# GuanxingLu/ManiGaussian

Hardware: AMD Instinct MI355X
Metric: Gaussians rasterized/sec (fwd+bwd), 128x128, 32 feat-ch; HBM GB/s vs peak (higher is better)
Workload: dtype f32

## Files before the change

### manigaussian_amd/csrc/mgs_render_dense.hip

```cpp
#include "mgs_render_common.h"

namespace mgs {

constexpr int TRACE_EVENTS = 24;
__device__ unsigned long long g_trace[512 * 16 * TRACE_EVENTS];
#define MGS_TRACE(ev)                                                                                      \
  do {                                                                                                     \
    if ((r.dbg & 256) && lane == 0 && blockIdx.x < 512 && (ev) < TRACE_EVENTS)                              \
      g_trace[((size_t)blockIdx.x * 16 + w) * TRACE_EVENTS + (ev)] = __builtin_amdgcn_s_memtime();         \
  } while (0)

template <int F, bool FAST, bool EXACT, int NW, int CHS, bool TWO>
__global__ void __launch_bounds__(NW * 64, TWO ? 4 : 1)
coop_fwd_pairs_kernel(RenderArgs r, const uint2* __restrict__ ranges, const uint32_t* __restrict__ point_list,
                      float* __restrict__ T_end, float* __restrict__ T_mid,
                      uint32_t* __restrict__ last_pos, float* __restrict__ partial, uint32_t* __restrict__ surv,
                      size_t surv_stride, uint2* __restrict__ nsurv, float* __restrict__ final_T,
                      uint32_t* __restrict__ last_chunk, float* __restrict__ out_color, float* __restrict__ out_feat,
                      uint32_t* __restrict__ round_base, uint32_t pool, uint32_t* __restrict__ flags, int nblocks,
                      uint64_t* host_status, uint32_t status_tag, unsigned long long* hs_fail_mark) {
  static_assert(CHS == 64, "a chunk is two 32-lane groups of the Gaussian-major backward");
  using f32x16 = __attribute__((ext_vector_type(16))) float;
  constexpr int NCH = F + 3;
  constexpr bool MF = F >= 16;
  constexpr int NT = MF ? (F + 31) / 32 : 0;
  constexpr int NVF = MF ? 0 : F;
  constexpr int NP = NW / 2;
  constexpr int NS = 2;
  constexpr int NSTEP = CHS / 2;
  constexpr int TRS = 33;
  constexpr int NOWN = (NCH + NW - 1) / NW;
  constexpr uint32_t ROUND = NW * CHS;
  constexpr uint32_t FSTEP = NW * 64;
  constexpr int FILLK = 3;
  constexpr int TRR = NT * 32 + 3;
  __shared__ float trs[MF ? NW * TRR * TRS : 1];
  __shared__ uint32_t lastcc[NW];
  __shared__ float4 recP[NW][CHS / 4 * 2 * 3];
  __shared__ uint32_t sid[NW * CHS];
  __shared__ float4 rowq[NW][NS][CHS];
  __shared__ float rowf[NVF > 0 ? NW * NS * CHS * NVF : 1];
  __shared__ float Tp[2][NW][64];
  __shared__ unsigned long long red_last[64];
  __shared__ uint32_t cnt[2][FILLK * NW];
  __shared__ uint32_t rbase[2];
  constexpr uint32_t RBH = 16;
  __shared__ uint32_t rb_hist[RBH];
  const int tid = threadIdx.x, lane = tid & 63;
  const int w = __builtin_amdgcn_readfirstlane(tid >> 6);
  if (blockIdx.x == 0 && tid == 0 && hs_fail_mark) *hs_fail_mark = 0ull;
  const int pr = w >> 1, hh = w & 1;
  const int k_ = lane >> 5, pl_ = lane & 31;
  int tile, sub;
  map_block(blockIdx.x, tile, sub);
  if (tile >= r.tiles_x * r.tiles_y) return;
  const PixBlk p = pix_blk(r, tile, sub, lane);
  const int pixq_ = 32 * hh + pl_;
  const int pixq = pixq_, k = k_, pl = pl_;
  const PixBlk pq = pix_blk(r, tile, sub, pixq);
  const int pixx_ = 32 * (hh ^ k) + pl;
  const int pixx = pixx_;
  const bool insidex = pix_blk(r, tile, sub, pixx).inside;
  const uint2 rng = ranges[tile];
  const bool use_feat = (F > 0) && r.include_feature;
  const auto feat_rsrc = __builtin_amdgcn_make_buffer_rsrc(const_cast<float*>(r.feats), 0, 0xffffffffu, 0x00020000);
  uint32_t* __restrict__ my_rounds = round_base + round_entry(rng.x, tile, sub, 0);
  bool overflow = false;
  uint32_t* my_surv = surv + (size_t)sub * surv_stride + rng.x;

  float Tround = 1.0f;
  uint32_t my_vis = 0;
  float my_Tf = 1.0f;
  if (w == 0) red_last[lane] = (unsigned long long)__float_as_uint(1.0f);
  uint32_t my_lastcc = 0xffffffffu;
  MGS_TRACE(0);

  uint32_t next = rng.x;
  uint32_t qhead = 0;
  uint32_t qtail = 0;
  uint32_t cbase = 0;
  uint32_t fill = 0;
  uint32_t round = 0;

  const bool allocator = tid == (NW - 1) * 64;
  const bool static0 = (uint32_t)nblocks <= 1024u && (uint32_t)nblocks * (uint32_t)NW <= pool;
  const uint32_t dyn_base = static0 ? (uint32_t)nblocks * (uint32_t)NW : 0u;
  for (;; round++) {
    int k = k_, pl = pl_, pixq = pixq_, pixx = pixx_;
    asm volatile("" : "+v"(k), "+v"(pl), "+v"(pixq), "+v"(pixx));
    uint32_t b0 = 0;
    const bool more = next < rng.y || qtail > qhead;
    if (allocator && more) {
      if (static0 && round == 0) b0 = ((uint32_t)tile * 4u + (uint32_t)sub) * (uint32_t)NW;
      else b0 = dyn_base + atomicAdd(&flags[FLAG_CHUNKS_USED], (uint32_t)NW);
    }
    while (qtail - qhead < ROUND && next < rng.y) {
      uint32_t idd[FILLK], rk[FILLK];
      float4 a0[FILLK], a1[FILLK];
      {
#pragma unroll
        for (int kf = 0; kf < FILLK; kf++) {
          const uint32_t e = next + (uint32_t)kf * FSTEP + (uint32_t)tid;
          idd[kf] = e < rng.y ? point_list[e] : 0xffffffffu;
        }
#pragma unroll
        for (int kf = 0; kf < FILLK; kf++) {
          a0[kf] = make_float4(0, 0, 0, 0); a1[kf] = make_float4(0, 0, -1.f, -1.f);
          if (idd[kf] != 0xffffffffu) { a0[kf] = r.rec[2 * (size_t)idd[kf]]; a1[kf] = r.rec[2 * (size_t)idd[kf] + 1]; }
        }
#pragma unroll
        for (int kf = 0; kf < FILLK; kf++) {
          const bool sk = idd[kf] != 0xffffffffu && cull_ok<EXACT>(a0[kf], a1[kf], p);
          const unsigned long long sm = ballot(sk);
          rk[kf] = sk ? (uint32_t)__builtin_popcountll(sm & ((1ull << lane) - 1ull)) : 0xffffffffu;
          if (lane == 0) cnt[fill & 1][kf * NW + w] = (uint32_t)__builtin_popcountll(sm);
        }
      }
      __syncthreads();
      const uint32_t v = lane < FILLK * NW ? cnt[fill & 1][lane] : 0u;
      const uint32_t incl = wave_incl_scan_add_u32(v);
      const uint32_t total = bcast_lane_u32(incl, 63);
#pragma unroll
      for (int kf = 0; kf < FILLK; kf++) {
        const uint32_t base = bcast_lane_u32(incl - v, kf * NW + w);
        if (rk[kf] != 0xffffffffu) {
          const uint32_t n = qtail + base + rk[kf];
          my_surv[n] = idd[kf];
          if (round == 0 && n < ROUND) {
            const uint32_t e = n & (CHS - 1);
            float* rp = reinterpret_cast<float*>(&recP[n / CHS][0]) + (((e >> 2) * 2 + (e & 1)) * 12 + ((e >> 1) & 1));
            rp[0] = a0[kf].x; rp[2] = a0[kf].y; rp[4] = a0[kf].z; rp[6] = a0[kf].w; rp[8] = a1[kf].x; rp[10] = a1[kf].y;
            sid[n] = idd[kf];
          }
        }
      }
      qtail += total;
      next += FILLK * FSTEP;
      fill++;
    }
    if (allocator && more) {
      rbase[round & 1] = b0;
      if (round < RBH) rb_hist[round] = b0;
      my_rounds[4 * (size_t)round] = b0;
    }
    MGS_TRACE(1 + 8 * round);
    __syncthreads();
    MGS_TRACE(2 + 8 * round);
    const uint32_t avail = qtail - qhead;
    const bool exhausted = !(next < rng.y);
    uint32_t nchunk = exhausted ? (avail + CHS - 1) / CHS : avail / CHS;
    nchunk = min(nchunk, (uint32_t)NW);
    if (nchunk == 0) break;

    struct Rec3 { float4 XY, CC, ZO; };
    auto rec3_of = [&](uint32_t buf, int j) -> Rec3 {
      return Rec3{recP[buf][(2 * j + k) * 3], recP[buf][(2 * j + k) * 3 + 1], recP[buf][(2 * j + k) * 3 + 2]};
    };
    auto alpha2_rec = [&](const Rec3& R) -> f32x2 {
      const float4 XY = R.XY, CC = R.CC, ZO = R.ZO;
      const f32x2 dx = f32x2{XY.x, XY.y} - pq.pxf, dy = f32x2{XY.z, XY.w} - pq.pyf;
      const f32x2 power = gauss_power2v(f32x2{CC.x, CC.y}, f32x2{CC.z, CC.w}, f32x2{ZO.x, ZO.y}, dx, dy);
      const f32x2 G = exp2_<FAST>(power);
      const f32x2 oG = f32x2{ZO.z, ZO.w} * G;
      const float a0 = fminf(0.99f, oG.x), a1 = fminf(0.99f, oG.y);
      return f32x2{((power.x > 0.0f) || (a0 < 1.0f / 255.0f)) ? 0.f : a0, ((power.y > 0.0f) || (a1 < 1.0f / 255.0f)) ? 0.f : a1};
    };
    auto alpha2_of = [&](uint32_t buf, int j) -> f32x2 { return alpha2_rec(rec3_of(buf, j)); };
    float al[NSTEP];
    uint32_t nmy[NS];
#pragma unroll
    for (int q = 0; q < NS; q++) {
      const uint32_t ci = (uint32_t)pr + (uint32_t)q * NP;
      const bool hasq = ci < nchunk;
      nmy[q] = hasq ? min((uint32_t)CHS, avail - ci * CHS) : 0u;
      if (q == 0) {
#pragma unroll
        for (int s = 0; s < NSTEP; s++) al[s] = 0.f;
      }
      float tp = 1.0f;
      if (hasq) {
        float4 rq = make_float4(0, 0, 0, __uint_as_float(0u));
        float fv[NVF > 0 ? NVF : 1];
#pragma unroll
        for (int i = 0; i < (NVF > 0 ? NVF : 1); i++) fv[i] = 0.f;
        const bool valid = (uint32_t)lane < nmy[q];
        float* rp = reinterpret_cast<float*>(&recP[ci][0]) + (((lane >> 2) * 2 + (lane & 1)) * 12 + ((lane >> 1) & 1));
        int tile_ = tile;
        asm volatile("" : "+s"(tile_));
        const uint32_t gbase = gauss_base(r, tile_);
        auto colour_row = [&](uint32_t id) {
          const uint32_t gid = gauss_of(gbase, id);
          const uint32_t cid = r.colors_per_view ? id : gid;
          rq = make_float4(r.colors[(size_t)cid * 3], r.colors[(size_t)cid * 3 + 1], r.colors[(size_t)cid * 3 + 2],
                           __uint_as_float(gid));
          if constexpr (NVF > 0) {
            if (use_feat) {
#pragma unroll
              for (int i = 0; i < NVF; i++) fv[i] = r.feats[(size_t)gid * F + i];
            }
          }
        };
        if (round == 0) {
          if (valid) {
            colour_row(sid[ci * CHS + (uint32_t)lane]);
          } else {
            rp[0] = 0.f; rp[2] = 0.f; rp[4] = 0.f; rp[6] = 0.f; rp[8] = 0.f; rp[10] = 0.f;
            rq.w = __uint_as_float(gauss_of(gbase, sid[ci * CHS]));
          }
        } else {
          float4 g0 = make_float4(0, 0, 0, 0), g1 = make_float4(0, 0, -1.f, -1.f);
          if (valid) {
            const uint32_t id = my_surv[qhead + ci * CHS + (uint32_t)lane];
            g0 = r.rec[2 * (size_t)id]; g1 = r.rec[2 * (size_t)id + 1];
            colour_row(id);
          } else {
            rq.w = __uint_as_float(gauss_of(gbase, my_surv[qhead + ci * CHS]));
          }
          rp[0] = g0.x; rp[2] = g0.y; rp[4] = g0.z; rp[6] = g0.w; rp[8] = g1.x;
          rp[10] = valid ? g1.y : 0.f;
        }
        wave_lds_sync();
        if (q == 0) MGS_TRACE(3 + 8 * round);
        f32x2 tp2 = {1.0f, 1.0f};
        Rec3 Rn = rec3_of(ci, 0);
#pragma unroll
        for (int j = 0; j < NSTEP / 2; j++) {
          const Rec3 Rc = Rn;
          if (j + 1 < NSTEP / 2) Rn = rec3_of(ci, j + 1);
          const f32x2 a2 = alpha2_rec(Rc);
          if (q == 0) { al[2 * j] = a2.x; al[2 * j + 1] = a2.y; }
          tp2 = tp2 * (1.0f - a2);
        }
        tp = tp2.x * tp2.y;
        rowq[w][q][lane] = rq;
        if constexpr (NVF > 0) {
#pragma unroll
          for (int i = 0; i < NVF; i++) rowf[(((size_t)w * NS + q) * CHS + lane) * NVF + i] = fv[i];
        }
        float t0 = tp, t1 = tp;
        swap32(t0, t1);
        tp = t0 * t1;
      }
      if (k == 0) Tp[round & 1][ci][pixq] = tp;
    }
    MGS_TRACE(4 + 8 * round);
    __syncthreads();
    __builtin_amdgcn_s_waitcnt(0x0F70);
    MGS_TRACE(5 + 8 * round);
    const uint32_t rb = rbase[round & 1];
    if (rb + (uint32_t)NW > pool) { overflow = true; break; }
    float Tin[NS], Tnext = Tround;
#pragma unroll
    for (int q = 0; q < NS; q++) Tin[q] = Tround;
#pragma unroll
    for (int c2 = 0; c2 < NW; c2++) {
      const float t2 = Tp[round & 1][c2][pixx];
#pragma unroll
      for (int q = 0; q < NS; q++) Tin[q] = (c2 < pr + q * NP) ? Tin[q] * t2 : Tin[q];
      Tnext *= t2;
    }
#pragma unroll
    for (int q = 0; q < NS; q++) {
      const uint32_t ci = (uint32_t)pr + (uint32_t)q * NP;
      const bool hasq = ci < nchunk;
      const float Tpart = __uint_as_float(lane_xor<32>(__float_as_uint(Tin[q]), lane));
      float T = k ? Tpart : Tin[q];
      const bool live = hasq && pq.inside && !(T < 0.0001f);
      if (ballot(live) != 0) {
        const uint32_t n_my = nmy[q];
        float Cc[3] = {0.f, 0.f, 0.f};
        float Cv[NVF > 0 ? NVF : 1];
#pragma unroll
        for (int i = 0; i < (NVF > 0 ? NVF : 1); i++) Cv[i] = 0.f;
        f32x16 acc[NT > 0 ? NT : 1];
#pragma unroll
        for (int t = 0; t < (NT > 0 ? NT : 1); t++)
#pragma unroll
          for (int i = 0; i < 16; i++) acc[t][i] = 0.f;
        constexpr int BD = 4;
        float Bq[NT > 0 ? NT : 1][BD];
        uint32_t gnext = __float_as_uint(rowq[w][q][k].w);
        auto load_B = [&](int s) {
          const uint32_t gide = gnext;
          if (s + 1 < NSTEP) gnext = __float_as_uint(rowq[w][q][2 * (s + 1) + k].w);
#pragma unroll
          for (int t = 0; t < (NT > 0 ? NT : 1); t++) {
            const int ch = 32 * t + pl;
            if constexpr (MF)
              Bq[t][s % BD] = __uint_as_float(__builtin_amdgcn_raw_buffer_load_b32(
                  feat_rsrc, gide * (uint32_t)(F * 4) + (uint32_t)((ch < F ? ch : 0) * 4), 0, 0));
          }
        };
        if constexpr (MF) {
#pragma unroll
          for (int s = 0; s < BD; s++) load_B(s);
        }
        float Tc = live ? T : 0.f;
        uint32_t last = 0;
        float Tm = T;
        bool stop = false;
        constexpr int GS = 4;
#pragma unroll
        for (int g = 0; g < NSTEP / GS; g++) {
          if (g * GS == NSTEP / 2) Tm = T;
          stop = stop || (uint32_t)(2 * g * GS) >= n_my || ballot(Tc != 0.f) == 0;
          __builtin_amdgcn_sched_barrier(0);
          if (!stop) {
            f32x2 a2q = {0.f, 0.f};
#pragma unroll
            for (int u4 = 0; u4 < GS; u4++) {
              const int s = g * GS + u4;
              if (q != 0 && (u4 & 1) == 0) a2q = alpha2_of(ci, s >> 1);
              float a0 = (q == 0) ? al[s] : ((u4 & 1) ? a2q.y : a2q.x), a1 = a0;
              swap32(a0, a1);
              float wq[2];
              const float aa[2] = {a0, a1};
#pragma unroll
              for (int u = 0; u < 2; u++) {
                const float test_T = Tc * (1.0f - aa[u]);
                const bool term = test_T < 0.0001f;
                wq[u] = (term ? 0.f : aa[u]) * Tc;
                Tc = term ? 0.f : test_T;
                T = term ? T : test_T;
                last = wq[u] > 0.f ? (uint32_t)(2 * s + u) + 1u : last;
              }
              const float wk = k ? wq[1] : wq[0];
              const float4 rq = rowq[w][q][2 * s + k];
              Cc[0] += rq.x * wk; Cc[1] += rq.y * wk; Cc[2] += rq.z * wk;
              if constexpr (NVF > 0) {
#pragma unroll
                for (int i = 0; i < NVF; i++) Cv[i] += rowf[(((size_t)w * NS + q) * CHS + 2 * s + k) * NVF + i] * wk;
              }
              if constexpr (MF) {
#pragma unroll
                for (int t = 0; t < NT; t++) {
                  float bv = Bq[t][s % BD];
                  if constexpr (F % 32 != 0) bv = (32 * t + pl) < F ? bv : 0.f;
                  acc[t] = __builtin_amdgcn_mfma_f32_32x32x2f32(wk, bv, acc[t], 0, 0, 0);
                }
                if (s + BD < NSTEP) load_B(s + BD);
              }
            }
          }
        }
        if constexpr (MF) {
#pragma unroll
          for (int t = 0; t < NT; t++)
#pragma unroll
            for (int i = 0; i < BD; i++) asm volatile("" ::"v"(Bq[t][i]));
        }
        if (last <= 32u) Tm = T;
#pragma unroll
        for (int i = 0; i < 3; i++) Cc[i] += __uint_as_float(lane_xor<32>(__float_as_uint(Cc[i]), lane));
#pragma unroll
        for (int i = 0; i < NVF; i++) Cv[i] += __uint_as_float(lane_xor<32>(__float_as_uint(Cv[i]), lane));
        MGS_TRACE(6 + 8 * round);
        const size_t slot = (size_t)rb + (size_t)ci;
        float* pp = partial + slot * NCH * 64 + pixq;
        if (k == 0) {
          T_end[slot * 64 + pixq] = T;
          T_mid[slot * 64 + pixq] = Tm;
          last_pos[slot * 64 + pixq] = last;
#pragma unroll
          for (int i = 0; i < 3; i++) pp[i * 64] = Cc[i];
#pragma unroll
          for (int i = 0; i < NVF; i++) pp[(3 + i) * 64] = Cv[i];
        }
        if constexpr (MF) {
          float* tb = trs + (size_t)w * TRR * TRS;
#pragma unroll
          for (int t = 0; t < NT; t++)
#pragma unroll
            for (int i = 0; i < 16; i++)
              tb[(32 * t + pl) * TRS + (i & 3) + 8 * (i >> 2) + 4 * k] = acc[t][i];
          if (k == 0) {
#pragma unroll
            for (int i = 0; i < 3; i++) tb[(NT * 32 + i) * TRS + pl] = Cc[i];
          }
          wave_lds_sync();
#pragma unroll
          for (int c = 0; c < F / 2; c++) {
            const int ch = k * (F / 2) + c;
            pp[(3 + ch) * 64] = tb[ch * TRS + pl];
          }
          wave_lds_sync();
          my_lastcc = cbase + ci;
        }
        if (live) { my_vis = cbase + ci + 1; my_Tf = T; }
      }
    }
    MGS_TRACE(7 + 8 * round);
    Tround = Tnext;
    qhead += min(avail, nchunk * CHS);
    cbase += nchunk;
    if (ballot(insidex && !(Tround < 0.0001f)) == 0) break;
  }

  MGS_TRACE(TRACE_EVENTS - 3);
  if (my_vis > 0 && k == 0)
    atomicMax(&red_last[pixq], ((unsigned long long)my_vis << 32) | (unsigned long long)__float_as_uint(my_Tf));
  if constexpr (MF) { if (lane == 0) lastcc[w] = my_lastcc; }
  __syncthreads();
  const unsigned long long rl = red_last[lane];
  const uint32_t vis = (uint32_t)(rl >> 32);
  const float Tf = __uint_as_float((uint32_t)rl);
  float img[NOWN];
#pragma unroll
  for (int kk = 0; kk < NOWN; kk++) img[kk] = 0.f;
  const uint32_t vmax = wave_umax(vis);
  constexpr int NFLY = 8;
  static_assert(NW % NFLY == 0, "a batch of the final sum lies inside one round");
  for (uint32_t c0 = 0; c0 < vmax; c0 += NFLY) {
    float v[NFLY][NOWN];
    const uint32_t rr = c0 / NW;
    uint32_t rb0 = rb_hist[rr < RBH ? rr : 0u];
    if (__builtin_expect(rr >= RBH, 0))
      rb0 = __hip_atomic_load(&my_rounds[4 * (size_t)rr], __ATOMIC_RELAXED, __HIP_MEMORY_SCOPE_WORKGROUP);
    rb0 = (uint32_t)__builtin_amdgcn_readfirstlane((int)rb0);
    bool inl[NFLY];
    unsigned long long needg = 0ull;
#pragma unroll
    for (int u = 0; u < NFLY; u++) {
      const uint32_t cc = c0 + u;
      inl[u] = false;
      if constexpr (MF) {
        const uint32_t ws = 2u * ((cc % NW) % NP) + (uint32_t)(lane >> 5);
        inl[u] = lastcc[ws] == cc;
      }
      needg |= ballot(cc < vis && !inl[u]);
#pragma unroll
      for (int kk = 0; kk < NOWN; kk++) v[u][kk] = 0.f;
    }
    if (needg != 0ull) {
#pragma unroll
      for (int u = 0; u < NFLY; u++) {
        const uint32_t cc = c0 + u;
        const bool gl = cc < vis && !inl[u];
        const size_t slot = gl ? (size_t)rb0 + (cc % NW) : 0;
        const float* pp = partial + slot * NCH * 64 + lane;
#pragma unroll
        for (int kk = 0; kk < NOWN; kk++) {
          const int ch = w + kk * NW;
          if (gl && ch < NCH && (ch < 3 || use_feat)) v[u][kk] = pp[ch * 64];
        }
      }
#pragma unroll
      for (int u = 0; u < NFLY; u++)
#pragma unroll
        for (int kk = 0; kk < NOWN; kk++) asm volatile("" : "+v"(v[u][kk]));
    }
    if constexpr (MF) {
#pragma unroll
      for (int u = 0; u < NFLY; u++) {
        const uint32_t cc = c0 + u;
        const uint32_t ws = 2u * ((cc % NW) % NP) + (uint32_t)(lane >> 5);
        const float* tb = trs + (size_t)ws * TRR * TRS + (lane & 31);
#pragma unroll
        for (int kk = 0; kk < NOWN; kk++) {
          const int ch = w + kk * NW;
          const int row = ch < 3 ? NT * 32 + ch : ch - 3;
          if (cc < vis && inl[u] && ch < NCH && (ch < 3 || use_feat)) v[u][kk] = tb[row * TRS];
        }
      }
    }
#pragma unroll
    for (int u = 0; u < NFLY; u++)
#pragma unroll
      for (int kk = 0; kk < NOWN; kk++) img[kk] += v[u][kk];
  }
  MGS_TRACE(TRACE_EVENTS - 2);
  uint32_t ticket = 0;
  if (tid == 0) {
    const uint32_t dep = overflow ? (atomicOr(&flags[FLAG_PREFILTERED], 0x100u) & 0u) : 0u;
    ticket = atomicAdd(&flags[FLAG_BLOCKS_DONE], 1u + dep) + 1u;
  }
  const size_t HW = (size_t)r.Hv * r.W;
  if (p.inside) {
#pragma unroll
    for (int kk = 0; kk < NOWN; kk++) {
      const int ch = w + kk * NW;
      if (ch < 3) out_color[((size_t)p.v * 3 + ch) * HW + p.pixl] = img[kk] + Tf * r.bg[ch];
      else if (ch < NCH && use_feat) out_feat[((size_t)p.v * F + (ch - 3)) * HW + p.pixl] = img[kk];
    }
  }
  if (w == 0) {
    last_chunk[((size_t)tile * 4 + sub) * 64 + lane] = vis;
    if (p.inside) final_T[p.pixa] = Tf;
    if (lane == 0) {
      nsurv[(size_t)tile * 4 + sub] = make_uint2(qtail, round > 0 || vis > 0 ? rb_hist[0] : 0u);
      if (ticket == (uint32_t)nblocks && host_status) {
        const uint32_t used = dyn_base + __hip_atomic_load(&flags[FLAG_CHUNKS_USED], __ATOMIC_RELAXED, __HIP_MEMORY_SCOPE_AGENT);
        const uint32_t ovf = (__hip_atomic_load(&flags[FLAG_PREFILTERED], __ATOMIC_RELAXED, __HIP_MEMORY_SCOPE_AGENT) >> 8) & 1u;
        __hip_atomic_store(host_status + 1, ((uint64_t)(status_tag & 0xffffu) << 48) | ((uint64_t)ovf << 32) | used,
                           __ATOMIC_RELEASE, __HIP_MEMORY_SCOPE_SYSTEM);
      }
    }
  }
  MGS_TRACE(TRACE_EVENTS - 1);
}

template <int F>
static hipError_t dense_F(const RenderArgs& r, const BinView& b, const ImgView& im, const ChunkView& cv, float* oc,
                          float* of, StatusSink st, hipStream_t s) {
  const int T = r.tiles_x * r.tiles_y;
  const int grid = ((T + 7) / 8) * 32;
#define MGS_CFD_(FAST, EXACT, NW, TWO)                                                                                \
  hipLaunchKernelGGL((coop_fwd_pairs_kernel<F, FAST, EXACT, NW, CHUNK, TWO>), dim3(grid), dim3(NW * 64), 0, s, r,      \
                     im.ranges, b.point_list, cv.T_end, cv.T_mid, cv.last_pos, cv.partial, cv.surv,                   \
                     cv.surv_stride, cv.nsurv, im.final_T, cv.last_chunk, oc, of, cv.round_base, cv.pool, im.flags,   \
                     4 * T, st.host, st.tag, (im.direct_keys && im.ready) ? im.ready + 1 : nullptr)
#define MGS_CFD(FAST, EXACT)                                                                                          \
  do {                                                                                                                \
    if constexpr (F > 32) MGS_CFD_(FAST, EXACT, 8, false);                               \
    else if (r.nwf == 8) MGS_CFD_(FAST, EXACT, 8, true);                                    \
    else MGS_CFD_(FAST, EXACT, 16, false);                                                                            \
  } while (0)
  if (r.fast_exp) { if (r.exact_cull) MGS_CFD(true, true); else MGS_CFD(true, false); }
  else            { if (r.exact_cull) MGS_CFD(false, true); else MGS_CFD(false, false); }
#undef MGS_CFD
#undef MGS_CFD_
  return hipGetLastError();
}

hipError_t launch_render_fwd_dense(const RenderArgs& r, const BinView& b, const ImgView& im, const ChunkView& cv,
                                   float* out_color, float* out_feat, StatusSink st, hipStream_t s) {
  const int F = r.include_feature ? r.F : 0;
  switch (F) {
#define X(N) case N: return dense_F<N>(r, b, im, cv, out_color, out_feat, st, s);
    MGS_FOR_EACH_F(X)
#undef X
    default: return hipErrorInvalidValue;
  }
}

}

extern "C" int mgs_debug_read_trace(unsigned long long* host, size_t count) {
  const size_t n = sizeof(mgs::g_trace) / sizeof(unsigned long long);
  return (int)hipMemcpyFromSymbol(host, HIP_SYMBOL(mgs::g_trace), (count < n ? count : n) * sizeof(unsigned long long));
}
```

Before: 753.9 million.

## Split per-round chunk processing into staged phases with early termination between pair groups

Measured after the change: 764.9 million, median of 6. 1.5% higher.

```diff
diff --git a/manigaussian_amd/csrc/mgs_render_dense.hip b/manigaussian_amd/csrc/mgs_render_dense.hip
--- a/manigaussian_amd/csrc/mgs_render_dense.hip
+++ b/manigaussian_amd/csrc/mgs_render_dense.hip
@@ -63,6 +63,7 @@
   const bool insidex = pix_blk(r, tile, sub, pixx).inside;
   const uint2 rng = ranges[tile];
   const bool use_feat = (F > 0) && r.include_feature;
+  const bool eager = (r.dbg & (1 << 17)) != 0;
   const auto feat_rsrc = __builtin_amdgcn_make_buffer_rsrc(const_cast<float*>(r.feats), 0, 0xffffffffu, 0x00020000);
   uint32_t* __restrict__ my_rounds = round_base + round_entry(rng.x, tile, sub, 0);
   bool overflow = false;
@@ -165,25 +166,23 @@
       const float a0 = fminf(0.99f, oG.x), a1 = fminf(0.99f, oG.y);
       return f32x2{((power.x > 0.0f) || (a0 < 1.0f / 255.0f)) ? 0.f : a0, ((power.y > 0.0f) || (a1 < 1.0f / 255.0f)) ? 0.f : a1};
     };
-    auto alpha2_of = [&](uint32_t buf, int j) -> f32x2 { return alpha2_rec(rec3_of(buf, j)); };
     float al[NSTEP];
     uint32_t nmy[NS];
 #pragma unroll
     for (int q = 0; q < NS; q++) {
       const uint32_t ci = (uint32_t)pr + (uint32_t)q * NP;
+      nmy[q] = ci < nchunk ? min((uint32_t)CHS, avail - ci * CHS) : 0u;
+    }
+    auto phase_a = [&](const int q, const bool publish) __attribute__((always_inline)) {
+      const uint32_t ci = (uint32_t)pr + (uint32_t)q * NP;
       const bool hasq = ci < nchunk;
-      nmy[q] = hasq ? min((uint32_t)CHS, avail - ci * CHS) : 0u;
-      if (q == 0) {
-#pragma unroll
-        for (int s = 0; s < NSTEP; s++) al[s] = 0.f;
-      }
       float tp = 1.0f;
       if (hasq) {
         float4 rq = make_float4(0, 0, 0, __uint_as_float(0u));
         float fv[NVF > 0 ? NVF : 1];
 #pragma unroll
         for (int i = 0; i < (NVF > 0 ? NVF : 1); i++) fv[i] = 0.f;
-        const bool valid = (uint32_t)lane < nmy[q];
+        const bool valid = (uint32_t)lane < (q ? nmy[1] : nmy[0]);
         float* rp = reinterpret_cast<float*>(&recP[ci][0]) + (((lane >> 2) * 2 + (lane & 1)) * 12 + ((lane >> 1) & 1));
         int tile_ = tile;
         asm volatile("" : "+s"(tile_));
@@ -228,7 +227,7 @@
           const Rec3 Rc = Rn;
           if (j + 1 < NSTEP / 2) Rn = rec3_of(ci, j + 1);
           const f32x2 a2 = alpha2_rec(Rc);
-          if (q == 0) { al[2 * j] = a2.x; al[2 * j + 1] = a2.y; }
+          al[2 * j] = a2.x; al[2 * j + 1] = a2.y;
           tp2 = tp2 * (1.0f - a2);
         }
         tp = tp2.x * tp2.y;
@@ -241,33 +240,17 @@
         swap32(t0, t1);
         tp = t0 * t1;
       }
-      if (k == 0) Tp[round & 1][ci][pixq] = tp;
-    }
-    MGS_TRACE(4 + 8 * round);
-    __syncthreads();
-    __builtin_amdgcn_s_waitcnt(0x0F70);
-    MGS_TRACE(5 + 8 * round);
-    const uint32_t rb = rbase[round & 1];
-    if (rb + (uint32_t)NW > pool) { overflow = true; break; }
-    float Tin[NS], Tnext = Tround;
-#pragma unroll
-    for (int q = 0; q < NS; q++) Tin[q] = Tround;
-#pragma unroll
-    for (int c2 = 0; c2 < NW; c2++) {
-      const float t2 = Tp[round & 1][c2][pixx];
-#pragma unroll
-      for (int q = 0; q < NS; q++) Tin[q] = (c2 < pr + q * NP) ? Tin[q] * t2 : Tin[q];
-      Tnext *= t2;
-    }
-#pragma unroll
-    for (int q = 0; q < NS; q++) {
+      if (publish && k == 0) Tp[round & 1][ci][pixq] = tp;
+    };
+    uint32_t rb = 0;
+    auto phase_b = [&](const int q, const float Tin_q) __attribute__((always_inline)) {
       const uint32_t ci = (uint32_t)pr + (uint32_t)q * NP;
       const bool hasq = ci < nchunk;
-      const float Tpart = __uint_as_float(lane_xor<32>(__float_as_uint(Tin[q]), lane));
-      float T = k ? Tpart : Tin[q];
+      const float Tpart = __uint_as_float(lane_xor<32>(__float_as_uint(Tin_q), lane));
+      float T = k ? Tpart : Tin_q;
       const bool live = hasq && pq.inside && !(T < 0.0001f);
       if (ballot(live) != 0) {
-        const uint32_t n_my = nmy[q];
+        const uint32_t n_my = q ? nmy[1] : nmy[0];
         float Cc[3] = {0.f, 0.f, 0.f};
         float Cv[NVF > 0 ? NVF : 1];
 #pragma unroll
@@ -306,12 +289,10 @@
           stop = stop || (uint32_t)(2 * g * GS) >= n_my || ballot(Tc != 0.f) == 0;
           __builtin_amdgcn_sched_barrier(0);
           if (!stop) {
-            f32x2 a2q = {0.f, 0.f};
 #pragma unroll
             for (int u4 = 0; u4 < GS; u4++) {
               const int s = g * GS + u4;
-              if (q != 0 && (u4 & 1) == 0) a2q = alpha2_of(ci, s >> 1);
-              float a0 = (q == 0) ? al[s] : ((u4 & 1) ? a2q.y : a2q.x), a1 = a0;
+              float a0 = al[s], a1 = a0;
               swap32(a0, a1);
               float wq[2];
               const float aa[2] = {a0, a1};
@@ -388,7 +369,45 @@
         }
         if (live) { my_vis = cbase + ci + 1; my_Tf = T; }
       }
-    }
+    };
+    constexpr int GA = 2;
+    static_assert(GA < NP, "slot 1 goes in two groups of pairs");
+    float Tnext = Tround;
+    int p0 = 0, p1 = NP;
+#pragma clang loop unroll(disable)
+    for (int st = eager ? -1 : 0;; st++) {
+      asm volatile("" : "+v"(k), "+v"(pl), "+v"(pixq), "+v"(pixx));
+      const int q = st == 0 ? 0 : 1;
+      const bool act = pr >= p0 && pr < p1;
+#pragma unroll
+      for (int s = 0; s < NSTEP; s++) al[s] = 0.f;
+      if (act) {
+        phase_a(q, st <= 0 || !eager);
+        if (st > 0) MGS_TRACE(8 + 8 * round);
+      }
+      if (st < 0) continue;
+      if (st == 0) MGS_TRACE(4 + 8 * round);
+      if (st == 0 || !eager) __syncthreads();
+      if (st == 0) {
+        __builtin_amdgcn_s_waitcnt(0x0F70);
+        MGS_TRACE(5 + 8 * round);
+        rb = rbase[round & 1];
+        if (rb + (uint32_t)NW > pool) { overflow = true; break; }
+      }
+      float Tin = Tnext;
+#pragma unroll
+      for (int c2 = 0; c2 < NP; c2++) {
+        const float t2 = (c2 >= p0 && c2 < p1) ? Tp[round & 1][q * NP + c2][pixx] : 1.0f;
+        Tin = (c2 < pr) ? Tin * t2 : Tin;
+        Tnext *= t2;
+      }
+      if (act) phase_b(q, Tin);
+      if (st == 2) break;
+      p0 = st == 0 ? 0 : GA;
+      p1 = st == 0 ? GA : NP;
+      if (!((uint32_t)(NP + p0) < nchunk) || ballot(insidex && !(Tnext < 0.0001f)) == 0) break;
+    }
+    if (overflow) break;
     MGS_TRACE(7 + 8 * round);
     Tround = Tnext;
     qhead += min(avail, nchunk * CHS);
@@ -475,17 +494,20 @@
     ticket = atomicAdd(&flags[FLAG_BLOCKS_DONE], 1u + dep) + 1u;
   }
   const size_t HW = (size_t)r.Hv * r.W;
-  if (p.inside) {
+  int lane_o = lane;
+  asm volatile("" : "+v"(lane_o));
+  const PixBlk po = pix_blk(r, tile, sub, lane_o);
+  if (po.inside) {
 #pragma unroll
     for (int kk = 0; kk < NOWN; kk++) {
       const int ch = w + kk * NW;
-      if (ch < 3) out_color[((size_t)p.v * 3 + ch) * HW + p.pixl] = img[kk] + Tf * r.bg[ch];
-      else if (ch < NCH && use_feat) out_feat[((size_t)p.v * F + (ch - 3)) * HW + p.pixl] = img[kk];
+      if (ch < 3) out_color[((size_t)po.v * 3 + ch) * HW + po.pixl] = img[kk] + Tf * r.bg[ch];
+      else if (ch < NCH && use_feat) out_feat[((size_t)po.v * F + (ch - 3)) * HW + po.pixl] = img[kk];
     }
   }
   if (w == 0) {
     last_chunk[((size_t)tile * 4 + sub) * 64 + lane] = vis;
-    if (p.inside) final_T[p.pixa] = Tf;
+    if (po.inside) final_T[po.pixa] = Tf;
     if (lane == 0) {
       nsurv[(size_t)tile * 4 + sub] = make_uint2(qtail, round > 0 || vis > 0 ? rb_hist[0] : 0u);
       if (ticket == (uint32_t)nblocks && host_status) {
```
